# ADVRHumanoids/mpc_fatigue

Hardware: NVIDIA B200
Metric: rollout_steps_per_s_with_jacobians (higher is better)
Workload: dtype f64

## Files before the change

### mpc_fatigue_b200/csrc/kernels_jvp2.cu

```cuda
#include <atomic>
#include <cstdlib>
#include <mutex>
#include <vector>

#include "derivs.cuh"
#include "launch.cuh"

namespace mpcf {

template <int N>
struct WsLayout {
    static constexpr int kTile = 32;
    static constexpr int kPlanes2 = 3 * N * N;
    static constexpr int kPlanes1 = 4 * N;
    static constexpr int kQd = 0, kQdd = N, kFd = 2 * N, kQ = 3 * N;
    static constexpr int kStageDoubles = (kPlanes2 + kPlanes1) * kTile;
    static constexpr unsigned kStageBytes = kStageDoubles * sizeof(double);
    static constexpr int kRingDoubles = (kPlanes2 + 3 * N) * kTile;
    static constexpr unsigned kRingBytes = kRingDoubles * sizeof(double);
    static constexpr int kUnitDoubles = 4 * (kPlanes2 + kPlanes1);
    static MPCF_DI size_t chunk(long tile, int s) { return ((size_t)tile * 4 + s) * kStageDoubles; }
};
size_t jvp_ws_doubles_per_unit(int n) { return (size_t)4 * (3 * n * n + 4 * n); }

// ... 104 lines not shown
#pragma unroll
    for (int i = 0; i < N; ++i) {
        q[i] = __ldcs(w + (W::kQ + i) * 32);
        qd[i] = __ldcs(w + (W::kQd + i) * 32);
        qdd[i] = __ldcs(w + (W::kQdd + i) * 32);
    }
    {
        const long lin = (long)blockIdx.y * gridDim.x + blockIdx.x + 2 * kSmCountHint;
        if (lin < 4l * gridDim.x) {
            const long lu2 = (lin % gridDim.x) * blockDim.x + threadIdx.x;
            if (lu2 < cnt) {
                const double *o2 = ws + W::chunk(lu2 / 32, (int)(lin / gridDim.x)) + (lu2 & 31);
#pragma unroll
                for (int i = 0; i < N; ++i) {
                    asm volatile("prefetch.global.L2 [%0];" ::"l"(o2 + (W::kPlanes2 + W::kQ + i) * 32));
                    asm volatile("prefetch.global.L2 [%0];" ::"l"(o2 + (W::kPlanes2 + W::kQd + i) * 32));
                    asm volatile("prefetch.global.L2 [%0];" ::"l"(o2 + (W::kPlanes2 + W::kQdd + i) * 32));
                }
#pragma unroll
                for (int r = 0; r < N; ++r)
#pragma unroll
                    for (int c = 0; c <= r; ++c) asm volatile("prefetch.global.L2 [%0];" ::"l"(o2 + (2 * N * N + r * N + c) * 32));
            }
        }
    }
    auto emit = [&](int mat, int r, int c, double v) { __stcs(o + (mat * N * N + r * N + c) * 32, v); };
    if (KSMEM) {
        extern __shared__ double k2_slab[];
        SharedLinkStore ks{k2_slab + threadIdx.x, (int)blockDim.x};
        CFromShared Cs{k2_slab + 18 * (N - 1) * blockDim.x + threadIdx.x, (int)blockDim.x};
#pragma unroll
        for (int r = 0; r < N; ++r)
#pragma unroll
            for (int c = 0; c <= r; ++c) cp_async8(Cs.base + (r * (r + 1) / 2 + c) * Cs.stride, o + (2 * N * N + r * N + c) * 32);
        FdDerivs<StaticModel<N, L>, L>::run_cols(m, q, qd, qdd, Cs, emit, ks);
    } else {
        LocalLinkStore<N> ks;
        CFromGlobal<N> Cs{o};
        FdDerivs<StaticModel<N, L>, L>::run_cols(m, q, qd, qdd, Cs, emit, ks);
    }
}

template <int N>
__global__ void __launch_bounds__(kThreads) k_fd_derivs(const __grid_constant__ StaticParams<N> P, long U, const double *q, const double *qd,
                                                       const double *tau, double *Ao, double *Bo, double *Co, int ntot, int c0)
{
    const StaticModel<N, N> m{P};
    const long u = (long)blockIdx.x * blockDim.x + threadIdx.x;
    if (u >= U) return;
    double a[N], b[N], c[N], qdd[N], Cv[N * (N + 1) / 2];
#pragma unroll
    for (int i = 0; i < N; ++i) { a[i] = q[i * U + u]; b[i] = qd[i * U + u]; c[i] = tau[i * U + u]; }
    Dyn<double, StaticModel<N, N>>::template fd_crba<N, true>(m, a, b, c, qdd, Cv);
    auto at = [&](int r, int cc) { return (size_t)((c0 + r) * ntot + c0 + cc) * U + u; };
#pragma unroll
    for (int r = 0; r < N; ++r)
#pragma unroll
        for (int cc = 0; cc < N; ++cc) Co[at(r, cc)] = Cv[r >= cc ? r * (r + 1) / 2 + cc : cc * (cc + 1) / 2 + r];
    auto cget = [&](int r, int cc) { return Cv[r * (r + 1) / 2 + cc]; };
    CFromRegisters<decltype(cget)> Cs{cget};
    auto emit = [&](int mat, int r, int cc, double v) { (mat == 0 ? Ao : Bo)[at(r, cc)] = v; };
    extern __shared__ double link_slab[];
    SharedLinkStore ks{link_slab + threadIdx.x, (int)blockDim.x};
    FdDerivs<StaticModel<N, N>, N>::run_cols(m, a, b, qdd, Cs, emit, ks);
#pragma unroll 1
    for (int r = 0; r < N; ++r)
#pragma unroll 1
        for (int cc = 0; cc < ntot; ++cc)
            if (cc < c0 || cc >= c0 + N) {
                const size_t k = (size_t)((c0 + r) * ntot + cc) * U + u;
                Ao[k] = 0.0; Bo[k] = 0.0; Co[k] = 0.0;
            }
}

template <int N>
__global__ void __launch_bounds__(kThreads) k_rnea_derivs(const __grid_constant__ StaticParams<N> P, long U, const double *q, const double *qd,
                                                         const double *qdd, double *Dq, double *Dv, double *Mo, int ntot, int c0)
{
    const StaticModel<N, N> m{P};
    const long u = (long)blockIdx.x * blockDim.x + threadIdx.x;
    if (u >= U) return;
    double a[N], b[N], c[N];
#pragma unroll
    for (int i = 0; i < N; ++i) { a[i] = q[i * U + u]; b[i] = qd[i * U + u]; c[i] = qdd ? qdd[i * U + u] : 0.0; }
    extern __shared__ double link_slab[];
    SharedLinkStore ks{link_slab + threadIdx.x, (int)blockDim.x};
    struct Hooks {
        double *Dq, *Dv, *Mo;
        long U, u;
        int ntot, c0;
        MPCF_DI size_t at(int r, int cc) const { return (size_t)((c0 + r) * ntot + c0 + cc) * U + u; }
        MPCF_DI void link(int, const double *, const double *) const {}
        MPCF_DI void pair(int k, int j, const LinkFwd &, const LinkFwd &, double dqkj, double dqjk, double dvkj, double dvjk, double mkj) const
        {
            Dq[at(k, j)] = dqkj;
            Dv[at(k, j)] = dvkj;
            Mo[at(k, j)] = mkj;
            if (j < k) {
                Dq[at(j, k)] = dqjk;
                Dv[at(j, k)] = dvjk;
                Mo[at(j, k)] = mkj;
            }
        }
    } hooks{Dq, Dv, Mo, U, u, ntot, c0};
    FdDerivs<StaticModel<N, N>, N>::run_id_stream(m, a, b, c, hooks, ks);
#pragma unroll 1
    for (int r = 0; r < N; ++r)
#pragma unroll 1
        for (int cc = 0; cc < ntot; ++cc)
            if (cc < c0 || cc >= c0 + N) {
                const size_t k = (size_t)((c0 + r) * ntot + cc) * U + u;
                Dq[k] = 0.0; Dv[k] = 0.0; Mo[k] = 0.0;
            }
}

template <int N, int NEE>
struct NodeEvalJvpHooks {
    static constexpr int NE = NEE > 0 ? NEE : 1;
    double *Dq, *Dv;
    long U, u;
    int ntot, c0;
    double wsign;
    int je[NE];
    double pl[NE][3], pf[NE][3], Wo[NE][6];
    MPCF_DI void link(int i, const double *R, const double *o)
    {
#pragma unroll
        for (int e = 0; e < NEE; ++e)
            if (je[e] == i) {
#pragma unroll
                for (int r = 0; r < 3; ++r) pf[e][r] = o[r] + R[3 * r] * pl[e][0] + R[3 * r + 1] * pl[e][1] + R[3 * r + 2] * pl[e][2];
                double t[3];
                cross3(pf[e], Wo[e], t);
#pragma unroll
                for (int r = 0; r < 3; ++r) Wo[e][3 + r] += t[r];
            }
    }
    MPCF_DI void hvec(const LinkFwd &Kj, int e, double *h) const
    {
        double t[3], dp[3];
        cross3(Kj.S + 3, pf[e], t);
#pragma unroll
        for (int r = 0; r < 3; ++r) dp[r] = Kj.S[r] + t[r];
        cross3(dp, Wo[e], h);
    }
    MPCF_DI void pair(int k, int j, const LinkFwd &Kk, const LinkFwd &Kj, double dqkj, double dqjk, double dvkj, double dvjk, double) const
    {
#pragma unroll
        for (int e = 0; e < NEE; ++e)
            if (k <= je[e]) {
                double hj[3];
                hvec(Kj, e, hj);
                double vkj = dot3(Kk.S + 3, hj);
                if (j < k) {
                    double x[6], hk[3];
                    mxm(Kj.S, Kk.S, x);
                    vkj += dot6(x, Wo[e]);
                    hvec(Kk, e, hk);
                    dqjk += wsign * dot3(Kj.S + 3, hk);
                }
                dqkj += wsign * vkj;
            }
        Dq[(size_t)((c0 + k) * ntot + c0 + j) * U + u] = dqkj;
        Dv[(size_t)((c0 + k) * ntot + c0 + j) * U + u] = dvkj;
        if (j < k) {
            Dq[(size_t)((c0 + j) * ntot + c0 + k) * U + u] = dqjk;
            Dv[(size_t)((c0 + j) * ntot + c0 + k) * U + u] = dvjk;
        }
    }
};

template <int N, int NEE>
__global__ void __launch_bounds__(kThreads) k_node_eval_jvp(const __grid_constant__ StaticParams<N> P, long U, EeArgs ee, double wsign,
                                                           const double *q, const double *qd, const double *qdd, const double *W,
                                                           double *Dq, double *Dv, int ntot, int c0)
{
    const StaticModel<N, N> m{P};
    const long u = (long)blockIdx.x * blockDim.x + threadIdx.x;
    if (u >= U) return;
    double a[N], b[N], c[N];
#pragma unroll
    for (int i = 0; i < N; ++i) { a[i] = q[i * U + u]; b[i] = qd[i * U + u]; c[i] = qdd ? qdd[i * U + u] : 0.0; }
    NodeEvalJvpHooks<N, NEE> hooks;
    hooks.Dq = Dq; hooks.Dv = Dv; hooks.U = U; hooks.u = u; hooks.ntot = ntot; hooks.c0 = c0; hooks.wsign = wsign;
#pragma unroll
    for (int e = 0; e < NEE; ++e) {
        const int j = e < ee.nee ? ee.f[e].joint - c0 : -1;
        hooks.je[e] = (e < ee.nee && ee.f[e].joint >= 0 && j >= 0 && j < N) ? j : -1;
#pragma unroll
        for (int r = 0; r < 3; ++r) { hooks.pl[e][r] = ee.f[e].p[r]; hooks.pf[e][r] = 0.0; }
#pragma unroll
        for (int r = 0; r < 6; ++r) hooks.Wo[e][r] = (hooks.je[e] >= 0) ? W[(long)(6 * e + r) * U + u] : 0.0;
    }
    extern __shared__ double link_slab[];
    SharedLinkStore ks{link_slab + threadIdx.x, (int)blockDim.x};
    FdDerivs<StaticModel<N, N>, N>::run_id_stream(m, a, b, c, hooks, ks);
#pragma unroll 1
    for (int r = 0; r < N; ++r)
#pragma unroll 1
        for (int cc = 0; cc < ntot; ++cc)
            if (cc < c0 || cc >= c0 + N) { Dq[(size_t)((c0 + r) * ntot + cc) * U + u] = 0.0; Dv[(size_t)((c0 + r) * ntot + cc) * U + u] = 0.0; }
}

struct RneaDerivsDualBody {
    template <class MP>
    static MPCF_DI void run(const MP &m, long u, long U, const double *q, const double *qd, const double *qdd, double *Dq, double *Dv,
                            double *Mo)
    {
        constexpr int UNR = MP::kStatic ? MP::MAXN : 1;
        const int n = m.n();
        const int d = blockIdx.y;
        Dual a[MP::MAXN], b[MP::MAXN], c[MP::MAXN], t[MP::MAXN];
#pragma unroll UNR
        for (int i = 0; i < n; ++i) {
            a[i] = Dual(q[i * U + u], d == i ? 1.0 : 0.0);
            b[i] = Dual(qd[i * U + u], d == n + i ? 1.0 : 0.0);
            c[i] = Dual(qdd ? qdd[i * U + u] : 0.0, d == 2 * n + i ? 1.0 : 0.0);
        }
        Dyn<Dual, MP>::rnea(m, a, b, c, t);
        double *out = d < n ? Dq : (d < 2 * n ? Dv : Mo);
        const int col = d % n;
#pragma unroll UNR
        for (int r = 0; r < n; ++r) out[(size_t)(r * n + col) * U + u] = t[r].d;
    }
};

struct FdDerivsDualBody {
    template <class MP>
    static MPCF_DI void run(const MP &m, long u, long U, const double *q, const double *qd, const double *tau, double *Ao, double *Bo,
                            double *Co)
    {
        constexpr int UNR = MP::kStatic ? MP::MAXN : 1;
        const int n = m.n();
        const int d = blockIdx.y;
        Dual a[MP::MAXN], b[MP::MAXN], c[MP::MAXN], t[MP::MAXN];
#pragma unroll UNR
        for (int i = 0; i < n; ++i) {
            a[i] = Dual(q[i * U + u], d == i ? 1.0 : 0.0);
            b[i] = Dual(qd[i * U + u], d == n + i ? 1.0 : 0.0);
            c[i] = Dual(tau[i * U + u], d == 2 * n + i ? 1.0 : 0.0);
        }
        Dyn<Dual, MP>::aba(m, a, b, c, t);
        double *out = d < n ? Ao : (d < 2 * n ? Bo : Co);
        const int col = d % n;
#pragma unroll UNR
        for (int r = 0; r < n; ++r) out[(size_t)(r * n + col) * U + u] = t[r].d;
    }
};

template <int N, int L>
struct ColumnState {
    double Xq[N], Xv[N], Xf[N], aq[N], av[N], af[N];
    int jq, jv, jt;
    bool isdt;
    double ktau;
    double xq1;

    MPCF_DI void set_tau(const StaticParams<N> &P, double tauj)
    {
        ktau = 0.0;
#pragma unroll
        for (int i = 0; i < N; ++i)
            if (i == jt) ktau = 2.0 * P.fat[i][1] * P.fat[i][2] * tauj;
    }
    MPCF_DI void init(int col)
    {
        jq = col < N ? col : -1;
        jv = (col >= N && col < 2 * N) ? col - N : -1;
        jt = (col >= 2 * N && col < 3 * N) ? col - 2 * N : -1;
        isdt = col == 3 * N;
#pragma unroll
        for (int i = 0; i < N; ++i) {
            Xq[i] = (i == jq) ? 1.0 : 0.0;
            Xv[i] = (i == jv) ? 1.0 : 0.0;
            Xf[i] = 0.0;
            aq[i] = Xq[i]; av[i] = Xv[i]; af[i] = 0.0;
        }
        xq1 = 0.0;
    }
    MPCF_DI void finish(const StaticParams<N> &P, int s, const double *w1, double h, const double *nv)
    {
        const double cs = s < 2 ? 0.5 : (s == 2 ? 1.0 : 0.0);
        const double wt = (s == 0 || s == 3) ? 1.0 / 6.0 : 1.0 / 3.0;
#pragma unroll
        for (int i = 0; i < N; ++i) {
            const double qds = w1[(WsLayout<N>::kQd + i) * 32];
            double kf = 2.0 * P.fat[i][1] * P.fat[i][3] * qds * Xv[i] - P.fat[i][0] * Xf[i];
            if (i == jt) kf += ktau;
            double yq = h * Xv[i], yf = h * kf, yv = h * nv[i];
            if (isdt) {
                yq += qds;
                yv += w1[(WsLayout<N>::kQdd + i) * 32];
                yf += w1[(WsLayout<N>::kFd + i) * 32];
            }
            aq[i] = fma(wt, yq, aq[i]);
            av[i] = fma(wt, yv, av[i]);
            af[i] = fma(wt, yf, af[i]);
            Xq[i] = ((i == jq) ? 1.0 : 0.0) + cs * yq;
            Xv[i] = ((i == jv) ? 1.0 : 0.0) + cs * yv;
            Xf[i] = cs * yf;
            if (s == 0 && (i == jq || i == jv)) xq1 = Xq[i];
        }
    }
    MPCF_DI void stage(const StaticParams<N> &P, int s, const double *w, double h)
    {
        double nv[N];
        if (s == 0) {
#pragma unroll
            for (int r = 0; r < N; ++r) {
                double kv = 0.0;
                if (jq >= 0 && jq / L == r / L) kv = w[(r * N + jq) * 32];
                if (jv >= 0 && jv / L == r / L) kv = w[(N * N + r * N + jv) * 32];
                nv[r] = kv;
            }
        } else if (s == 1 && !isdt) {
            const int js = jq >= 0 ? jq : jv;
#pragma unroll
            for (int r = 0; r < N; ++r) {
                double kv = 0.0;
                if (js >= 0 && js / L == r / L) kv = w[(r * N + js) * 32] * xq1;
#pragma unroll
                for (int c = 0; c < N; ++c) {
                    if (r / L != c / L) continue;
                    kv = fma(w[(N * N + r * N + c) * 32], Xv[c], kv);
                }
                nv[r] = kv;
            }
        } else {
#pragma unroll
            for (int r = 0; r < N; ++r) {
                double kv = 0.0;
#pragma unroll
                for (int c = 0; c < N; ++c) {
                    if (r / L != c / L) continue;
                    kv = fma(w[(r * N + c) * 32], Xq[c], kv);
                    kv = fma(w[(N * N + r * N + c) * 32], Xv[c], kv);
                }
                nv[r] = kv;
            }
        }
        if (jt >= 0) {
#pragma unroll
            for (int r = 0; r < N; ++r)
                if (jt / L == r / L) nv[r] += w[(2 * N * N + r * N + jt) * 32];
        }
        finish(P, s, w + 3 * N * N * 32, h, nv);
    }
    static MPCF_DI void stage2(ColumnState &a, ColumnState &b, const StaticParams<N> &P, int s, const double *w, double h)
    {
        double na[N], nb[N];
#pragma unroll
        for (int r = 0; r < N; ++r) {
            double ka = 0.0, kb = 0.0;
#pragma unroll
            for (int c = 0; c < N; ++c) {
                if (r / L != c / L) continue;
                const double A = w[(r * N + c) * 32], B = w[(N * N + r * N + c) * 32];
                ka = fma(A, a.Xq[c], ka);
                kb = fma(A, b.Xq[c], kb);
                ka = fma(B, a.Xv[c], ka);
                kb = fma(B, b.Xv[c], kb);
            }
            if (a.jt >= 0 && a.jt / L == r / L) ka += w[(2 * N * N + r * N + a.jt) * 32];
            if (b.jt >= 0 && b.jt / L == r / L) kb += w[(2 * N * N + r * N + b.jt) * 32];
            na[r] = ka;
            nb[r] = kb;
        }
        a.finish(P, s, w + 3 * N * N * 32, h, na);
        b.finish(P, s, w + 3 * N * N * 32, h, nb);
    }
    template <bool WHOLE>
    MPCF_DI void store(const StaticParams<N> &P, int col, double h, long U, long u, double *jac, int ntot_, int c0_) const
    {
        const int ntot = WHOLE ? N : ntot_, c0 = WHOLE ? 0 : c0_;
        const long PC = 4 * ntot + 1;
        const long ocol = isdt ? 4 * ntot : (col / N) * ntot + c0 + col % N;
#pragma unroll
        for (int i = 0; i < N; ++i) {
            __stcs(jac + ((size_t)(c0 + i) * PC + ocol) * U + u, aq[i]);
            __stcs(jac + ((size_t)(ntot + c0 + i) * PC + ocol) * U + u, av[i]);
            __stcs(jac + ((size_t)(2 * ntot + c0 + i) * PC + ocol) * U + u, af[i]);
        }
        if (isdt) {
#pragma unroll
            for (int j = 0; j < N; ++j) {
                const double z = P.fat[j][0] * h;
                const double g = 1.0 + z * (-1.0 + z * (0.5 + z * (-1.0 / 6.0 + z * (1.0 / 24.0))));
                if (WHOLE) {
#pragma unroll
                    for (int r = 0; r < 3 * N; ++r) __stcs(jac + ((size_t)r * PC + 3 * N + j) * U + u, (r == 2 * N + j) ? g : 0.0);
                } else {
#pragma unroll
                    for (int blk = 0; blk < 3; ++blk)
#pragma unroll
                        for (int i = 0; i < N; ++i)
                            __stcs(jac + ((size_t)(blk * ntot + c0 + i) * PC + 3 * ntot + c0 + j) * U + u, (blk == 2 && i == j) ? g : 0.0);
                }
            }
        }
    }
};

template <int N, int L>
__global__ void __launch_bounds__(kThreads) k_step_vjp(const __grid_constant__ StaticParams<N> P, long U, long u0, long cnt,
                                                      const double *__restrict__ tau, double dt, const double *__restrict__ dt_u,
                                                      const VjpArgs a, int gdt_add, const double *__restrict__ ws)
{
    static_assert(N == L, "the reverse sweep runs one serial chain at a time (forests: one launch per chain)");
    using W = WsLayout<N>;
    const long lu = (long)blockIdx.x * blockDim.x + threadIdx.x;
    if (lu >= cnt) return;
    const long u = u0 + lu;
    const double h = dt_u ? dt_u[u] : dt;
    double lam[3 * N], gx[3 * N], ad[3 * N], gt[N], kt[N];
#pragma unroll
    for (int i = 0; i < N; ++i) {
        lam[i] = a.lq ? a.lq[i * a.ldl + u] : 0.0;
        lam[N + i] = a.lqd ? a.lqd[i * a.ldl + u] : 0.0;
        lam[2 * N + i] = a.lf ? a.lf[i * a.ldl + u] : 0.0;
        gx[i] = lam[i] + (a.aq ? a.aq[i * a.lda + u] : 0.0);
        gx[N + i] = lam[N + i] + (a.aqd ? a.aqd[i * a.lda + u] : 0.0);
        gx[2 * N + i] = lam[2 * N + i] + (a.af ? a.af[i * a.lda + u] : 0.0);
        kt[i] = 2.0 * P.fat[i][1] * P.fat[i][2] * tau[i * U + u];
        gt[i] = 0.0;
    }
#pragma unroll
    for (int i = 0; i < 3 * N; ++i) ad[i] = 0.0;
    double gh = 0.0;
#pragma unroll 1
    for (int s = 3; s >= 0; --s) {
        const double cs = s < 2 ? 0.5 : (s == 2 ? 1.0 : 0.0);
        const double wt = (s == 0 || s == 3) ? 1.0 / 6.0 : 1.0 / 3.0;
        const double *w = ws + W::chunk(lu / 32, s) + (lu & 31);
        const double *v = w + W::kPlanes2 * 32;
        double rq[N], rv[N], rf[N], nq[N], nv[N];
#pragma unroll
        for (int i = 0; i < N; ++i) {
            const double qds = __ldcs(v + (W::kQd + i) * 32);
            const double pq = fma(wt, lam[i], cs * ad[i]), pv = fma(wt, lam[N + i], cs * ad[N + i]),
                         pf = fma(wt, lam[2 * N + i], cs * ad[2 * N + i]);
            gh = fma(pq, qds, gh);
            gh = fma(pv, __ldcs(v + (W::kQdd + i) * 32), gh);
            gh = fma(pf, __ldcs(v + (W::kFd + i) * 32), gh);
            rq[i] = h * pq;
            rv[i] = h * pv;
            rf[i] = h * pf;
            nq[i] = 0.0;
            nv[i] = fma(2.0 * P.fat[i][1] * P.fat[i][3] * qds, rf[i], rq[i]);
            gt[i] = fma(kt[i], rf[i], gt[i]);
        }
#pragma unroll
        for (int r = 0; r < N; ++r) {
            if (P.fence0 > r) continue;
            const double x = rv[r];
#pragma unroll
            for (int c = 0; c < N; ++c) {
                nq[c] = fma(__ldcs(w + (r * N + c) * 32), x, nq[c]);
                nv[c] = fma(__ldcs(w + (N * N + r * N + c) * 32), x, nv[c]);
                gt[c] = fma(__ldcs(w + (2 * N * N + r * N + c) * 32), x, gt[c]);
            }
        }
#pragma unroll
        for (int i = 0; i < N; ++i) {
            ad[i] = nq[i];
            ad[N + i] = nv[i];
            ad[2 * N + i] = -P.fat[i][0] * rf[i];
            gx[i] += ad[i];
            gx[N + i] += ad[N + i];
            gx[2 * N + i] += ad[2 * N + i];
        }
    }
#pragma unroll
    for (int i = 0; i < N; ++i) {
        a.gq[i * a.ldg + u] = gx[i];
        a.gqd[i * a.ldg + u] = gx[N + i];
        a.gf[i * a.ldg + u] = gx[2 * N + i];
        a.gtau[i * a.ldgt + u] = gt[i];
    }
    if (a.gdt) a.gdt[u] = gdt_add ? a.gdt[u] + gh : gh;
}

MPCF_DI unsigned smem_u32(const void *p) { return (unsigned)__cvta_generic_to_shared(p); }
MPCF_DI void mbar_init(unsigned long long *bar, unsigned count)
{
    asm volatile("mbarrier.init.shared::cta.b64 [%0], %1;" ::"r"(smem_u32(bar)), "r"(count) : "memory");
}
MPCF_DI void mbar_arrive(unsigned long long *bar)
{
    asm volatile("{\n\t.reg .b64 st;\n\tmbarrier.arrive.shared::cta.b64 st, [%0];\n\t}" ::"r"(smem_u32(bar)) : "memory");
}
MPCF_DI void mbar_arrive_expect_tx(unsigned long long *bar, unsigned bytes)
{
    asm volatile("{\n\t.reg .b64 st;\n\tmbarrier.arrive.expect_tx.release.cta.shared::cta.b64 st, [%0], %1;\n\t}" ::"r"(smem_u32(bar)), "r"(bytes)
                 : "memory");
}
MPCF_DI void mbar_wait(unsigned long long *bar, unsigned parity)
{
    unsigned done;
    do {
        asm volatile("{\n\t.reg .pred p;\n\tmbarrier.try_wait.parity.shared::cta.b64 p, [%1], %2;\n\tselp.b32 %0, 1, 0, p;\n\t}"
                     : "=r"(done)
                     : "r"(smem_u32(bar)), "r"(parity)
                     : "memory");
    } while (!done);
}
MPCF_DI void bulk_g2s(void *dst, const void *src, unsigned bytes, unsigned long long *bar)
{
    asm volatile("cp.async.bulk.shared::cluster.global.mbarrier::complete_tx::bytes [%0], [%1], %2, [%3];" ::"r"(smem_u32(dst)), "l"(src),
                 "r"(bytes), "r"(smem_u32(bar))
                 : "memory");
}

template <class W, int NBUF>
MPCF_DI void tma_issue(unsigned item, double *buf, unsigned long long *full, unsigned long long *empty, const double *ws, unsigned bid,
                       unsigned nblk)
{
    const unsigned slot = item % NBUF, round = item / NBUF;
    const long t = bid + (long)(item / 4) * nblk;
    mbar_wait(&empty[slot], (round & 1) ^ 1);
    mbar_arrive_expect_tx(&full[slot], W::kRingBytes);
    bulk_g2s(buf + (size_t)slot * W::kRingDoubles, ws + W::chunk(t, item & 3), W::kRingBytes, &full[slot]);
}

template <int N, int L, int NBUF, int CPW, bool WHOLE>
__global__ void __launch_bounds__(32 * ((3 * N + CPW) / CPW), 1)
    k_chain_rule_tma(const __grid_constant__ StaticParams<N> P, long U, long u0, long cnt, const double *__restrict__ tau, long UT, double dt,
                     const double *__restrict__ dt_u, const double *__restrict__ ws, double *__restrict__ jac, long UJ, int ntot, int c0)
{
    using W = WsLayout<N>;
    constexpr int NC = 3 * N + 1;
    constexpr int NW = (NC + CPW - 1) / CPW;
    extern __shared__ __align__(128) unsigned char smem_raw[];
    double *buf = reinterpret_cast<double *>(smem_raw);
    unsigned long long *full = reinterpret_cast<unsigned long long *>(smem_raw + (size_t)NBUF * W::kRingBytes);
    unsigned long long *empty = full + NBUF;
    const int warp = threadIdx.x >> 5, lane = threadIdx.x & 31;
    const long ntiles = (cnt + 31) / 32;
    const long my_tiles = blockIdx.x < ntiles ? (ntiles - blockIdx.x + gridDim.x - 1) / gridDim.x : 0;
    const unsigned nitems = (unsigned)(my_tiles * 4);
    const bool producer = threadIdx.x == 0;
    if (producer) {
        for (int i = 0; i < NBUF; ++i) { mbar_init(&full[i], 1); mbar_init(&empty[i], NW); }
        asm volatile("fence.mbarrier_init.release.cluster;" ::: "memory");
        for (unsigned i = 0; i < NBUF - 1 && i < nitems; ++i)
            tma_issue<W, NBUF>(i, buf, full, empty, ws, blockIdx.x, gridDim.x);
    }
    __syncthreads();
    const int col0 = warp, col1 = warp + NW;
    const bool two = CPW == 2 && col1 < NC;
    unsigned it = 0;
    for (long t = blockIdx.x; t < ntiles; t += gridDim.x) {
        const long lu = t * 32 + lane;
        const bool live = lu < cnt;
        const long u = u0 + (live ? lu : 0);
        const double h = dt_u ? dt_u[u] : dt;
        ColumnState<N, L> a, b;
        a.init(col0);
        a.set_tau(P, a.jt >= 0 ? tau[(size_t)a.jt * UT + u] : 0.0);
        if (CPW == 2) {
            b.init(two ? col1 : col0);
            b.set_tau(P, b.jt >= 0 ? tau[(size_t)b.jt * UT + u] : 0.0);
        }
#pragma unroll 1
        for (int s = 0; s < 4; ++s, ++it) {
            if (producer && it + NBUF - 1 < nitems) tma_issue<W, NBUF>(it + NBUF - 1, buf, full, empty, ws, blockIdx.x, gridDim.x);
            const unsigned slot = it % NBUF, round = it / NBUF;
            mbar_wait(&full[slot], round & 1);
            const double *w = buf + (size_t)slot * W::kRingDoubles + lane;
            if (CPW == 2) ColumnState<N, L>::stage2(a, b, P, s, w, h);
            else a.stage(P, s, w, h);
            __syncwarp();
            if (lane == 0) mbar_arrive(&empty[slot]);
        }
        if (live) {
            a.template store<WHOLE>(P, col0, h, UJ, u, jac, ntot, c0);
            if (two) b.template store<WHOLE>(P, col1, h, UJ, u, jac, ntot, c0);
        }
    }
}

template <int N, int L, int NCY>
__global__ void __launch_bounds__(32 * NCY, 2)
    k_chain_rule_ldg(const __grid_constant__ StaticParams<N> P, long U, long u0, long cnt, const double *__restrict__ tau, long UT, double dt,
                     const double *__restrict__ dt_u, const double *__restrict__ ws, double *__restrict__ jac, long UJ, int ntot, int c0)
{
    using W = WsLayout<N>;
    const long lu = (long)blockIdx.x * 32 + threadIdx.x;
    if (lu >= cnt) return;
    const long u = u0 + lu;
    const double h = dt_u ? dt_u[u] : dt;
    constexpr int NC = 3 * N + 1;
    for (int col = threadIdx.y; col < NC; col += blockDim.y) {
        ColumnState<N, L> st;
        st.init(col);
        st.set_tau(P, st.jt >= 0 ? tau[(size_t)st.jt * UT + u] : 0.0);
#pragma unroll 1
        for (int s = 0; s < 4; ++s) st.stage(P, s, ws + W::chunk(blockIdx.x, s) + threadIdx.x, h);
        st.template store<false>(P, col, h, UJ, u, jac, ntot, c0);
    }
}

struct ProfEvent { cudaEvent_t a, b; int k; };
static std::atomic<bool> g_prof_on{false};
static std::mutex g_prof_mu;
static std::vector<ProfEvent> g_prof;
void jvp_profile_enable(bool on) { g_prof_on.store(on); }
static cudaEvent_t prof_begin(int k, cudaStream_t s)
{
    if (!g_prof_on.load(std::memory_order_relaxed)) return nullptr;
    ProfEvent e;
    cudaEventCreate(&e.a);
    cudaEventCreate(&e.b);
    e.k = k;
    cudaEventRecord(e.a, s);
    std::lock_guard<std::mutex> lk(g_prof_mu);
    g_prof.push_back(e);
    return e.b;
}
static void prof_end(cudaEvent_t b, cudaStream_t s)
{
    if (b) cudaEventRecord(b, s);
}
int jvp_profile_read(double *ms3, long *launches)
{
    std::lock_guard<std::mutex> lk(g_prof_mu);
    ms3[0] = ms3[1] = ms3[2] = 0.0;
    *launches = (long)g_prof.size();
    for (auto &e : g_prof) {
        float t = 0.f;
        cudaEventSynchronize(e.b);
        cudaEventElapsedTime(&t, e.a, e.b);
        ms3[e.k] += t;
        cudaEventDestroy(e.a);
        cudaEventDestroy(e.b);
    }
    g_prof.clear();
    return 0;
}

static int current_device()
{
    int dev = 0;
    cudaGetDevice(&dev);
    return dev >= 0 && dev < 64 ? dev : 0;
}
static int sm_count()
{
    static int n[64] = {};
    const int dev = current_device();
    if (!n[dev]) {
        cudaDeviceGetAttribute(&n[dev], cudaDevAttrMultiProcessorCount, dev);
        if (n[dev] <= 0) n[dev] = 148;
    }
    return n[dev];
}

template <int N, int L>
struct K2Config {
    static constexpr int kThreadsK2 = (2 * (18 * (N - 1) + N * (N + 1) / 2) * kThreads * (int)sizeof(double) <= 227 * 1024) ? kThreads : 96;
    static constexpr int kSlab = (18 * (N - 1) + N * (N + 1) / 2) * kThreadsK2 * (int)sizeof(double);
    static constexpr bool kSmem = N == L && 2 * kSlab <= 227 * 1024;
};

template <int N, int L>
static void launch_stages_derivs(const StaticParams<N> &P, long U, long u0, long cnt, const double *q, const double *qd, const double *tau,
                                 const double *theat, long UT, const double *f, double dt, const double *dt_u, double *qn, double *qdn,
                                 double *fn, double *ws, cudaStream_t s)
{
    using K2 = K2Config<N, L>;
    const unsigned gb = (unsigned)((cnt + kThreads - 1) / kThreads);
    cudaEvent_t pe = prof_begin(0, s);
    k_step_stages<N, L><<<gb, kThreads, 0, s>>>(P, U, u0, cnt, q, qd, tau, theat, UT, f, dt, dt_u, qn, qdn, fn, ws);
    prof_end(pe, s);
    pe = prof_begin(1, s);
    static const int k2smem = getenv("MPCF_K2_SMEM") ? atoi(getenv("MPCF_K2_SMEM")) : 1;
    bool k2done = false;
    if constexpr (K2::kSmem) {
        if (k2smem) {
            k_stage_derivs<N, L, true><<<dim3((unsigned)((cnt + K2::kThreadsK2 - 1) / K2::kThreadsK2), 4), K2::kThreadsK2, K2::kSlab, s>>>(P, cnt, ws);
            k2done = true;
        }
    }
    if (!k2done) k_stage_derivs<N, L, false><<<dim3(gb, 4), kThreads, 0, s>>>(P, cnt, ws);
    prof_end(pe, s);
}

template <int N, int L>
static cudaError_t run_jvp2(const StaticParams<N> &P, long U, long Ucnt, const double *q, const double *qd, const double *tau, const double *theat,
                            long UT, const double *f,
                            double dt, const double *dt_u, double *qn, double *qdn, double *fn, double *jac, long UJ, double *ws, long Uc,
                            cudaStream_t s, int ntot = N, int c0 = 0)
{
    using W = WsLayout<N>;
    constexpr bool kTma = N <= 7;
    constexpr int kRingMax = (227 * 1024 - 256) / (int)W::kRingBytes;
    constexpr int NBUF = kTma ? (kRingMax > 5 ? 5 : kRingMax) : 0;
    constexpr int kCpwDefault = (3 * N + 1 <= 19) ? 1 : 2;
    constexpr size_t smem = (size_t)NBUF * W::kRingBytes + 2 * NBUF * sizeof(unsigned long long);
    using K2 = K2Config<N, L>;
    constexpr bool kK2Smem = K2::kSmem;
    if constexpr (kTma) {
        static std::atomic<bool> attr_set[64];
        const int dev = current_device();
        if (!attr_set[dev].load(std::memory_order_acquire)) {
            cudaError_t e = cudaSuccess;
            if constexpr (kCpwDefault == 1) {
                e = cudaFuncSetAttribute(k_chain_rule_tma<N, L, NBUF, 1, true>, cudaFuncAttributeMaxDynamicSharedMemorySize, (int)smem);
                if (e != cudaSuccess) return e;
                e = cudaFuncSetAttribute(k_chain_rule_tma<N, L, NBUF, 1, false>, cudaFuncAttributeMaxDynamicSharedMemorySize, (int)smem);
                if (e != cudaSuccess) return e;
            }
            e = cudaFuncSetAttribute(k_chain_rule_tma<N, L, NBUF, 2, true>, cudaFuncAttributeMaxDynamicSharedMemorySize, (int)smem);
            if (e != cudaSuccess) return e;
            e = cudaFuncSetAttribute(k_chain_rule_tma<N, L, NBUF, 2, false>, cudaFuncAttributeMaxDynamicSharedMemorySize, (int)smem);
            if (e != cudaSuccess) return e;
            if constexpr (kK2Smem) {
                e = cudaFuncSetAttribute(k_stage_derivs<N, L, true>, cudaFuncAttributeMaxDynamicSharedMemorySize, K2::kSlab);
                if (e != cudaSuccess) return e;
            }
            attr_set[dev].store(true, std::memory_order_release);
        }
    }
    for (long u0 = 0; u0 < Ucnt; u0 += Uc) {
        const long cnt = (Ucnt - u0) < Uc ? (Ucnt - u0) : Uc;
        const long ntiles = (cnt + 31) / 32;
        launch_stages_derivs<N, L>(P, U, u0, cnt, q, qd, tau, theat, UT, f, dt, dt_u, qn, qdn, fn, ws, s);
        cudaEvent_t pe = prof_begin(2, s);
        if constexpr (kTma) {
            const unsigned g3 = (unsigned)(ntiles < sm_count() ? ntiles : sm_count());
            static const int cpw_env = getenv("MPCF_K3_CPW") ? atoi(getenv("MPCF_K3_CPW")) : 1;
            const int cpw = kCpwDefault == 2 ? 2 : cpw_env;
            if (cpw == 2) {
                (ntot == N ? k_chain_rule_tma<N, L, NBUF, 2, true> : k_chain_rule_tma<N, L, NBUF, 2, false>)<<<g3, 32 * ((3 * N + 2) / 2), smem, s>>>(
                    P, U, u0, cnt, theat, UT, dt, dt_u, ws, jac, UJ, ntot, c0);
            } else if constexpr (kCpwDefault == 1) {
                (ntot == N ? k_chain_rule_tma<N, L, NBUF, 1, true> : k_chain_rule_tma<N, L, NBUF, 1, false>)<<<g3, 32 * (3 * N + 1), smem, s>>>(
                    P, U, u0, cnt, theat, UT, dt, dt_u, ws, jac, UJ, ntot, c0);
            }
        } else {
            k_chain_rule_ldg<N, L, 10><<<(unsigned)ntiles, dim3(32, 10), 0, s>>>(P, U, u0, cnt, theat, UT, dt, dt_u, ws, jac, UJ, ntot, c0);
        }
        prof_end(pe, s);
        g_launches.fetch_add(3);
    }
    return cudaGetLastError();
}

template <int L, class V>
__global__ void __launch_bounds__(256) k_forest_fill_cross(int ntot, long cntv, long UJ, double *jac)
{
    const long uv = (long)blockIdx.x * blockDim.x + threadIdx.x;
    if (uv >= cntv) return;
    const int r = blockIdx.y, rc = (r % ntot) / L, nch = ntot / L;
    const long PC = 4 * ntot + 1;
    V zero;
    memset(&zero, 0, sizeof(V));
    double *row = jac + (size_t)r * PC * UJ;
    for (int b = 0; b < 4; ++b)
        for (int oc = 0; oc < nch; ++oc) {
            if (oc == rc) continue;
            double *p = row + (size_t)(b * ntot + oc * L) * UJ;
#pragma unroll
            for (int i = 0; i < L; ++i) __stcs(reinterpret_cast<V *>(p + (size_t)i * UJ) + uv, zero);
        }
}

template <int L>
static cudaError_t run_forest(const LaunchModel &m, long U, long Ucnt, const double *q, const double *qd, const double *tau, const double *theat,
                              long UT, const double *f, double dt,
                              const double *dt_u, double *qn, double *qdn, double *fn, double *jac, long UJ, double *ws, long Uc, cudaStream_t s)
{
    const StaticParams<L> *cp = static_cast<const StaticParams<L> *>(m.chain_params);
    for (int c = 0; c < m.n / L; ++c) {
        const size_t off = (size_t)c * L * U;
        cudaError_t e = run_jvp2<L, L>(cp[c], U, Ucnt, q + off, qd + off, tau + off, theat + (size_t)c * L * UT, UT, f + off, dt, dt_u, qn ? qn + off : nullptr,
                                       qdn ? qdn + off : nullptr, fn ? fn + off : nullptr, jac, UJ, ws, Uc, s, m.n, L * c);
        if (e != cudaSuccess) return e;
    }
    if (Ucnt % 2 == 0 && UJ % 2 == 0 && (reinterpret_cast<size_t>(jac) & 15) == 0)
        k_forest_fill_cross<L, double2><<<dim3((unsigned)((Ucnt / 2 + 255) / 256), 3 * m.n), 256, 0, s>>>(m.n, Ucnt / 2, UJ, jac);
    else
        k_forest_fill_cross<L, double><<<dim3((unsigned)((Ucnt + 255) / 256), 3 * m.n), 256, 0, s>>>(m.n, Ucnt, UJ, jac);
    g_launches.fetch_add(1);
    return cudaGetLastError();
}

bool jvp2_supported(const LaunchModel &m) { return family_chain_len(m.fam) > 0; }

cudaError_t launch_step_jvp_ws(const LaunchModel &m, long U, const double *q, const double *qd, const double *tau, const double *f,
                               double dt, const double *dt_u, double *qn, double *qdn, double *fn, double *jac, double *ws,
                               size_t ws_bytes, cudaStream_t s, long cnt, long UJ, const double *theat, long UT)
{
    if (!theat) { theat = tau; UT = U; }
    if (cnt < 0) cnt = U;
    if (UJ <= 0) UJ = U;
    if (cnt <= 0) return cudaSuccess;
    const size_t per_unit = jvp_ws_doubles_per_unit(family_chain_len(m.fam)) * sizeof(double);
    long Uc = (long)(ws_bytes / per_unit);
    Uc -= Uc % 32;
    if (Uc < 32) return cudaErrorInvalidValue;
    switch (m.fam) {
    case FAM_CHAIN3:
        return run_jvp2<3, 3>(*static_cast<const StaticParams<3> *>(m.static_params), U, cnt, q, qd, tau, theat, UT, f, dt, dt_u, qn, qdn, fn, jac, UJ, ws, Uc, s);
    case FAM_CHAIN6:
        return run_jvp2<6, 6>(*static_cast<const StaticParams<6> *>(m.static_params), U, cnt, q, qd, tau, theat, UT, f, dt, dt_u, qn, qdn, fn, jac, UJ, ws, Uc, s);
    case FAM_CHAIN7:
        return run_jvp2<7, 7>(*static_cast<const StaticParams<7> *>(m.static_params), U, cnt, q, qd, tau, theat, UT, f, dt, dt_u, qn, qdn, fn, jac, UJ, ws, Uc, s);
    case FAM_FOREST12x6:
        return run_forest<6>(m, U, cnt, q, qd, tau, theat, UT, f, dt, dt_u, qn, qdn, fn, jac, UJ, ws, Uc, s);
    case FAM_FOREST14x7:
        return run_forest<7>(m, U, cnt, q, qd, tau, theat, UT, f, dt, dt_u, qn, qdn, fn, jac, UJ, ws, Uc, s);
    default:
        return cudaErrorInvalidValue;
    }
}

template <int N, int L>
static cudaError_t run_vjp2(const StaticParams<N> &P, long U, long Ucnt, const double *q, const double *qd, const double *tau, const double *f,
                            double dt, const double *dt_u, const VjpArgs &a, int gdt_add, double *qn, double *qdn, double *fn, double *ws, long Uc,
                            cudaStream_t s)
{
    using K2 = K2Config<N, L>;
    if constexpr (K2::kSmem) {
        static std::atomic<bool> attr_set[64];
        const int dev = current_device();
        if (!attr_set[dev].load(std::memory_order_acquire)) {
            const cudaError_t e = cudaFuncSetAttribute(k_stage_derivs<N, L, true>, cudaFuncAttributeMaxDynamicSharedMemorySize, K2::kSlab);
            if (e != cudaSuccess) return e;
            attr_set[dev].store(true, std::memory_order_release);
        }
    }
    for (long u0 = 0; u0 < Ucnt; u0 += Uc) {
        const long cnt = (Ucnt - u0) < Uc ? (Ucnt - u0) : Uc;
        launch_stages_derivs<N, L>(P, U, u0, cnt, q, qd, tau, tau, U, f, dt, dt_u, qn, qdn, fn, ws, s);
        k_step_vjp<N, L><<<(unsigned)((cnt + kThreads - 1) / kThreads), kThreads, 0, s>>>(P, U, u0, cnt, tau, dt, dt_u, a, gdt_add, ws);
        g_launches.fetch_add(3);
    }
    return cudaGetLastError();
}

template <int L>
static cudaError_t vjp_chains(const LaunchModel &m, long U, long cnt, const double *q, const double *qd, const double *tau, const double *f,
                              double dt, const double *dt_u, const VjpArgs &a, double *qn, double *qdn, double *fn, double *ws, long Uc,
                              cudaStream_t s)
{
    const StaticParams<L> *cp = static_cast<const StaticParams<L> *>(m.n == L ? m.static_params : m.chain_params);
    for (int c = 0; c < m.n / L; ++c) {
        const size_t off = (size_t)c * L * U;
        const cudaError_t e = run_vjp2<L, L>(cp[c], U, cnt, q + off, qd + off, tau + off, f + off, dt, dt_u, a.rows(c * L), c > 0,
                                             qn ? qn + off : nullptr, qdn ? qdn + off : nullptr, fn ? fn + off : nullptr, ws, Uc, s);
        if (e != cudaSuccess) return e;
    }
    return cudaSuccess;
}

cudaError_t launch_step_vjp_ws(const LaunchModel &m, long U, long cnt, const double *q, const double *qd, const double *tau, const double *f,
                               double dt, const double *dt_u, const VjpArgs &a, double *qn, double *qdn, double *fn, double *ws,
                               size_t ws_bytes, cudaStream_t s)
{
    if (cnt <= 0) return cudaSuccess;
    const size_t per_unit = jvp_ws_doubles_per_unit(family_chain_len(m.fam)) * sizeof(double);
    long Uc = (long)(ws_bytes / per_unit);
    Uc -= Uc % 32;
    if (Uc < 32) return cudaErrorInvalidValue;
    switch (family_chain_len(m.fam)) {
    case 3: return vjp_chains<3>(m, U, cnt, q, qd, tau, f, dt, dt_u, a, qn, qdn, fn, ws, Uc, s);
    case 6: return vjp_chains<6>(m, U, cnt, q, qd, tau, f, dt, dt_u, a, qn, qdn, fn, ws, Uc, s);
    case 7: return vjp_chains<7>(m, U, cnt, q, qd, tau, f, dt, dt_u, a, qn, qdn, fn, ws, Uc, s);
    default: return cudaErrorInvalidValue;
    }
}

static constexpr int link_slab_bytes(int n) { return 18 * (n - 1) * kThreads * (int)sizeof(double); }

template <int L>
static cudaError_t node_eval_jvp_chains(const LaunchModel &m, const EeArgs &ee, double wsign, long U, const double *q, const double *qd,
                                        const double *qdd, const double *W, double *dtau_dq, double *dtau_dqd, cudaStream_t s)
{
    const unsigned gb = (unsigned)((U + kThreads - 1) / kThreads);
    const StaticParams<L> *cp = static_cast<const StaticParams<L> *>(m.n == L ? m.static_params : m.chain_params);
    for (int c = 0; c < m.n / L; ++c) {
        const size_t off = (size_t)c * L * U;
        auto go = [&](auto kern) {
            cudaError_t e = cudaFuncSetAttribute(kern, cudaFuncAttributeMaxDynamicSharedMemorySize, link_slab_bytes(L));
            if (e != cudaSuccess) return e;
            kern<<<gb, kThreads, link_slab_bytes(L), s>>>(cp[c], U, ee, wsign, q + off, qd + off, qdd ? qdd + off : nullptr, W, dtau_dq, dtau_dqd,
                                                         m.n, c * L);
            return cudaSuccess;
        };
        const cudaError_t e = ee.nee == 0 ? go(k_node_eval_jvp<L, 0>) : ee.nee == 1 ? go(k_node_eval_jvp<L, 1>)
                              : ee.nee == 2 ? go(k_node_eval_jvp<L, 2>) : go(k_node_eval_jvp<L, MPCF_MAX_EE>);
        if (e != cudaSuccess) return e;
        g_launches.fetch_add(1);
    }
    return cudaGetLastError();
}

cudaError_t launch_node_eval_jvp(const LaunchModel &m, const EeArgs &ee, double wsign, long U, const double *q, const double *qd,
                                 const double *qdd, const double *W, double *dtau_dq, double *dtau_dqd, cudaStream_t s)
{
    if (U <= 0) return cudaSuccess;
    switch (family_chain_len(m.fam)) {
    case 3: return node_eval_jvp_chains<3>(m, ee, wsign, U, q, qd, qdd, W, dtau_dq, dtau_dqd, s);
    case 6: return node_eval_jvp_chains<6>(m, ee, wsign, U, q, qd, qdd, W, dtau_dq, dtau_dqd, s);
    case 7: return node_eval_jvp_chains<7>(m, ee, wsign, U, q, qd, qdd, W, dtau_dq, dtau_dqd, s);
    default: return launch_node_eval_jvp_dual(m, ee, wsign, U, q, qd, qdd, W, dtau_dq, dtau_dqd, s);
    }
}

template <int L>
static cudaError_t rnea_derivs_chains(const LaunchModel &m, long U, const double *q, const double *qd, const double *qdd, double *Dq, double *Dv,
                                      double *M, cudaStream_t s)
{
    const unsigned gb = (unsigned)((U + kThreads - 1) / kThreads);
    const StaticParams<L> *cp = static_cast<const StaticParams<L> *>(m.n == L ? m.static_params : m.chain_params);
    const cudaError_t e = cudaFuncSetAttribute(k_rnea_derivs<L>, cudaFuncAttributeMaxDynamicSharedMemorySize, link_slab_bytes(L));
    if (e != cudaSuccess) return e;
    for (int c = 0; c < m.n / L; ++c) {
        const size_t off = (size_t)c * L * U;
        k_rnea_derivs<L><<<gb, kThreads, link_slab_bytes(L), s>>>(cp[c], U, q + off, qd + off, qdd ? qdd + off : nullptr, Dq, Dv, M, m.n, c * L);
        g_launches.fetch_add(1);
    }
    return cudaGetLastError();
}

cudaError_t launch_rnea_derivs(const LaunchModel &m, long U, const double *q, const double *qd, const double *qdd, double *Dq, double *Dv,
                               double *M, cudaStream_t s)
{
    if (U <= 0) return cudaSuccess;
    switch (family_chain_len(m.fam)) {
    case 3: return rnea_derivs_chains<3>(m, U, q, qd, qdd, Dq, Dv, M, s);
    case 6: return rnea_derivs_chains<6>(m, U, q, qd, qdd, Dq, Dv, M, s);
    case 7: return rnea_derivs_chains<7>(m, U, q, qd, qdd, Dq, Dv, M, s);
    default: return dispatch_generic<RneaDerivsDualBody>(m, U, 3 * m.n, s, q, qd, qdd, Dq, Dv, M);
    }
}

template <int L>
static cudaError_t fd_derivs_chains(const LaunchModel &m, long U, const double *q, const double *qd, const double *tau, double *A, double *B,
                                    double *C, cudaStream_t s)
{
    const unsigned gb = (unsigned)((U + kThreads - 1) / kThreads);
    const StaticParams<L> *cp = static_cast<const StaticParams<L> *>(m.n == L ? m.static_params : m.chain_params);
    const cudaError_t e = cudaFuncSetAttribute(k_fd_derivs<L>, cudaFuncAttributeMaxDynamicSharedMemorySize, link_slab_bytes(L));
    if (e != cudaSuccess) return e;
    for (int c = 0; c < m.n / L; ++c) {
        const size_t off = (size_t)c * L * U;
        k_fd_derivs<L><<<gb, kThreads, link_slab_bytes(L), s>>>(cp[c], U, q + off, qd + off, tau + off, A, B, C, m.n, c * L);
        g_launches.fetch_add(1);
    }
    return cudaGetLastError();
}

cudaError_t launch_fd_derivs(const LaunchModel &m, long U, const double *q, const double *qd, const double *tau, double *A, double *B,
                             double *C, cudaStream_t s)
{
    if (U <= 0) return cudaSuccess;
    switch (family_chain_len(m.fam)) {
    case 3: return fd_derivs_chains<3>(m, U, q, qd, tau, A, B, C, s);
    case 6: return fd_derivs_chains<6>(m, U, q, qd, tau, A, B, C, s);
    case 7: return fd_derivs_chains<7>(m, U, q, qd, tau, A, B, C, s);
    default: return dispatch_generic<FdDerivsDualBody>(m, U, 3 * m.n, s, q, qd, tau, A, B, C);
    }
}

}
```

Measured before the change: 226.0 million.

## Fuse stage-derivative and chain-rule kernels for six-joint serial chains

New measurement: 240.1 million, median of 6. 6.3% higher.

```diff
diff --git a/mpc_fatigue_b200/csrc/kernels_jvp2.cu b/mpc_fatigue_b200/csrc/kernels_jvp2.cu
--- a/mpc_fatigue_b200/csrc/kernels_jvp2.cu
+++ b/mpc_fatigue_b200/csrc/kernels_jvp2.cu
@@ -430,7 +430,9 @@
             if (s == 0 && (i == jq || i == jv)) xq1 = Xq[i];
         }
     }
-    MPCF_DI void stage(const StaticParams<N> &P, int s, const double *w, double h)
+    MPCF_DI void stage(const StaticParams<N> &P, int s, const double *w, double h) { stage(P, s, w, CFromGlobal<N>{w}, w + 3 * N * N * 32, h); }
+    template <class CM>
+    MPCF_DI void stage(const StaticParams<N> &P, int s, const double *w, const CM &Cm, const double *wv, double h)
     {
         double nv[N];
         if (s == 0) {
@@ -470,9 +472,9 @@
         if (jt >= 0) {
 #pragma unroll
             for (int r = 0; r < N; ++r)
-                if (jt / L == r / L) nv[r] += w[(2 * N * N + r * N + jt) * 32];
-        }
-        finish(P, s, w + 3 * N * N * 32, h, nv);
+                if (jt / L == r / L) nv[r] += Cm(r, jt);
+        }
+        finish(P, s, wv, h, nv);
     }
     static MPCF_DI void stage2(ColumnState &a, ColumnState &b, const StaticParams<N> &P, int s, const double *w, double h)
     {
@@ -497,7 +499,7 @@
         a.finish(P, s, w + 3 * N * N * 32, h, na);
         b.finish(P, s, w + 3 * N * N * 32, h, nb);
     }
-    template <bool WHOLE>
+    template <bool WHOLE, bool FCOLS = true>
     MPCF_DI void store(const StaticParams<N> &P, int col, double h, long U, long u, double *jac, int ntot_, int c0_) const
     {
         const int ntot = WHOLE ? N : ntot_, c0 = WHOLE ? 0 : c0_;
@@ -509,21 +511,26 @@
             __stcs(jac + ((size_t)(ntot + c0 + i) * PC + ocol) * U + u, av[i]);
             __stcs(jac + ((size_t)(2 * ntot + c0 + i) * PC + ocol) * U + u, af[i]);
         }
-        if (isdt) {
-#pragma unroll
-            for (int j = 0; j < N; ++j) {
-                const double z = P.fat[j][0] * h;
-                const double g = 1.0 + z * (-1.0 + z * (0.5 + z * (-1.0 / 6.0 + z * (1.0 / 24.0))));
-                if (WHOLE) {
-#pragma unroll
-                    for (int r = 0; r < 3 * N; ++r) __stcs(jac + ((size_t)r * PC + 3 * N + j) * U + u, (r == 2 * N + j) ? g : 0.0);
-                } else {
-#pragma unroll
-                    for (int blk = 0; blk < 3; ++blk)
-#pragma unroll
-                        for (int i = 0; i < N; ++i)
-                            __stcs(jac + ((size_t)(blk * ntot + c0 + i) * PC + 3 * ntot + c0 + j) * U + u, (blk == 2 && i == j) ? g : 0.0);
-                }
+        if (FCOLS && isdt) fatigue_cols<WHOLE>(P, h, U, u, jac, ntot, c0);
+    }
+    template <bool WHOLE>
+    static MPCF_DI void fatigue_cols(const StaticParams<N> &P, double h, long U, long u, double *jac, int ntot_, int c0_)
+    {
+        const int ntot = WHOLE ? N : ntot_, c0 = WHOLE ? 0 : c0_;
+        const long PC = 4 * ntot + 1;
+#pragma unroll
+        for (int j = 0; j < N; ++j) {
+            const double z = P.fat[j][0] * h;
+            const double g = 1.0 + z * (-1.0 + z * (0.5 + z * (-1.0 / 6.0 + z * (1.0 / 24.0))));
+            if (WHOLE) {
+#pragma unroll
+                for (int r = 0; r < 3 * N; ++r) __stcs(jac + ((size_t)r * PC + 3 * N + j) * U + u, (r == 2 * N + j) ? g : 0.0);
+            } else {
+#pragma unroll
+                for (int blk = 0; blk < 3; ++blk)
+#pragma unroll
+                    for (int i = 0; i < N; ++i)
+                        __stcs(jac + ((size_t)(blk * ntot + c0 + i) * PC + 3 * ntot + c0 + j) * U + u, (blk == 2 && i == j) ? g : 0.0);
             }
         }
     }
@@ -728,6 +735,111 @@
     }
 }
 
+template <int N>
+struct FusedLayout {
+    static constexpr int kLinkPlanes = 18 * (N - 1);
+    static constexpr int kTri = N * (N + 1) / 2;
+    static constexpr int kSlab = (kLinkPlanes + kTri) * kThreads * (int)sizeof(double);
+    static constexpr int kStage = (2 * N * N + 3 * N) * 32;
+    static constexpr bool kFits = 4 * kStage <= kLinkPlanes * kThreads;
+};
+
+template <int N, int L, bool WHOLE>
+__global__ void __launch_bounds__(kThreads) k_stage_derivs_chain(const __grid_constant__ StaticParams<N> P, long U, long u0, long cnt,
+                                                                 const double *__restrict__ tau, long UT, double dt, const double *__restrict__ dt_u,
+                                                                 double *ws, double *__restrict__ jac, long UJ, int ntot, int c0)
+{
+    static_assert(N == L && FusedLayout<N>::kFits, "one serial chain whose four stages fit the link slab");
+    static_assert(kThreads == 128, "one warp per RK4 stage");
+    const StaticModel<N, L> m{P};
+    using W = WsLayout<N>;
+    using F = FusedLayout<N>;
+    extern __shared__ __align__(128) double fused_slab[];
+    __shared__ unsigned long long full[4];
+    const int s = threadIdx.x >> 5, lane = threadIdx.x & 31;
+    const long lu = (long)blockIdx.x * 32 + lane;
+    const bool live = lu < cnt;
+    const int lc = live ? lane : (int)((cnt - 1) & 31);
+    double *o = ws + W::chunk(blockIdx.x, s) + lane;
+    const double *in = ws + W::chunk(blockIdx.x, s) + lc;
+    if (threadIdx.x == 0) {
+#pragma unroll
+        for (int i = 0; i < 4; ++i) mbar_init(&full[i], 1);
+        asm volatile("fence.mbarrier_init.release.cluster;" ::: "memory");
+    }
+    double q[N], qd[N], qdd[N];
+#pragma unroll
+    for (int i = 0; i < N; ++i) {
+        q[i] = __ldcs(in + (W::kPlanes2 + W::kQ + i) * 32);
+        qd[i] = __ldcs(in + (W::kPlanes2 + W::kQd + i) * 32);
+        qdd[i] = __ldcs(in + (W::kPlanes2 + W::kQdd + i) * 32);
+    }
+    {
+        const long t2 = (long)blockIdx.x + 2 * kSmCountHint;
+        const long lu2 = t2 * 32 + lane;
+        if (t2 < gridDim.x && lu2 < cnt) {
+            const double *o2 = ws + W::chunk(t2, s) + lane;
+#pragma unroll
+            for (int i = 0; i < 4 * N; ++i) asm volatile("prefetch.global.L2 [%0];" ::"l"(o2 + (W::kPlanes2 + i) * 32));
+#pragma unroll
+            for (int r = 0; r < N; ++r)
+#pragma unroll
+                for (int c = 0; c <= r; ++c) asm volatile("prefetch.global.L2 [%0];" ::"l"(o2 + (2 * N * N + r * N + c) * 32));
+        }
+    }
+    CFromShared Cs{fused_slab + F::kLinkPlanes * kThreads + threadIdx.x, kThreads};
+    {
+        SharedLinkStore ks{fused_slab + threadIdx.x, kThreads};
+#pragma unroll
+        for (int r = 0; r < N; ++r)
+#pragma unroll
+            for (int c = 0; c <= r; ++c) cp_async8(Cs.base + (r * (r + 1) / 2 + c) * kThreads, in + (2 * N * N + r * N + c) * 32);
+        auto emit = [&](int mat, int r, int c, double v) { o[(mat * N * N + r * N + c) * 32] = v; };
+        FdDerivs<StaticModel<N, L>, L>::run_cols(m, q, qd, qdd, Cs, emit, ks);
+    }
+    asm volatile("fence.proxy.async;" ::: "memory");
+    __syncthreads();
+    if (threadIdx.x == 0) {
+        asm volatile("fence.proxy.async;" ::: "memory");
+#pragma unroll
+        for (int st = 0; st < 4; ++st) {
+            const double *src = ws + W::chunk(blockIdx.x, st);
+            double *dst = fused_slab + st * F::kStage;
+            mbar_arrive_expect_tx(&full[st], F::kStage * (unsigned)sizeof(double));
+            bulk_g2s(dst, src, 2 * N * N * 32 * (unsigned)sizeof(double), &full[st]);
+            bulk_g2s(dst + 2 * N * N * 32, src + W::kPlanes2 * 32, 3 * N * 32 * (unsigned)sizeof(double), &full[st]);
+        }
+    }
+    constexpr int NC = 3 * N + 1;
+    const long u = u0 + (long)blockIdx.x * 32 + lc;
+    const double h = dt_u ? dt_u[u] : dt;
+#pragma unroll 1
+    for (int col = s; col < NC; col += 4) {
+        ColumnState<N, L> a;
+        a.init(col);
+        a.set_tau(P, a.jt >= 0 ? tau[(size_t)a.jt * UT + u] : 0.0);
+#pragma unroll 1
+        for (int st = 0; st < 4; ++st) {
+            mbar_wait(&full[st], 0);
+            const CFromShared Ct{fused_slab + F::kLinkPlanes * kThreads + st * 32 + lane, kThreads};
+            auto Cm = [&](int r, int c) { return r >= c ? Ct(r, c) : Ct(c, r); };
+            const double *w = fused_slab + st * F::kStage + lane;
+            a.stage(P, st, w, Cm, w + 2 * N * N * 32, h);
+        }
+        if (live) a.template store<WHOLE, false>(P, col, h, UJ, u, jac, ntot, c0);
+    }
+}
+
+template <int N, bool WHOLE>
+__global__ void __launch_bounds__(kThreads) k_fatigue_cols(const __grid_constant__ StaticParams<N> P, long u0, long cnt, double dt,
+                                                           const double *__restrict__ dt_u, double *jac, long UJ, int ntot, int c0)
+{
+    const long lu = (long)blockIdx.x * blockDim.x + threadIdx.x;
+    if (lu >= cnt) return;
+    const long u = u0 + lu;
+    ColumnState<N, N>::template fatigue_cols<WHOLE>(P, dt_u ? dt_u[u] : dt, UJ, u, jac, ntot, c0);
+}
+
 struct ProfEvent { cudaEvent_t a, b; int k; };
 static std::atomic<bool> g_prof_on{false};
 static std::mutex g_prof_mu;
@@ -791,16 +903,25 @@
 };
 
 template <int N, int L>
+static void launch_step_stages(const StaticParams<N> &P, long U, long u0, long cnt, const double *q, const double *qd, const double *tau,
+                               const double *theat, long UT, const double *f, double dt, const double *dt_u, double *qn, double *qdn,
+                               double *fn, double *ws, cudaStream_t s)
+{
+    cudaEvent_t pe = prof_begin(0, s);
+    k_step_stages<N, L><<<(unsigned)((cnt + kThreads - 1) / kThreads), kThreads, 0, s>>>(P, U, u0, cnt, q, qd, tau, theat, UT, f, dt, dt_u, qn,
+                                                                                      qdn, fn, ws);
+    prof_end(pe, s);
+}
+
+template <int N, int L>
 static void launch_stages_derivs(const StaticParams<N> &P, long U, long u0, long cnt, const double *q, const double *qd, const double *tau,
                                  const double *theat, long UT, const double *f, double dt, const double *dt_u, double *qn, double *qdn,
                                  double *fn, double *ws, cudaStream_t s)
 {
     using K2 = K2Config<N, L>;
     const unsigned gb = (unsigned)((cnt + kThreads - 1) / kThreads);
-    cudaEvent_t pe = prof_begin(0, s);
-    k_step_stages<N, L><<<gb, kThreads, 0, s>>>(P, U, u0, cnt, q, qd, tau, theat, UT, f, dt, dt_u, qn, qdn, fn, ws);
-    prof_end(pe, s);
-    pe = prof_begin(1, s);
+    launch_step_stages<N, L>(P, U, u0, cnt, q, qd, tau, theat, UT, f, dt, dt_u, qn, qdn, fn, ws, s);
+    cudaEvent_t pe = prof_begin(1, s);
     static const int k2smem = getenv("MPCF_K2_SMEM") ? atoi(getenv("MPCF_K2_SMEM")) : 1;
     bool k2done = false;
     if constexpr (K2::kSmem) {
@@ -827,6 +948,7 @@
     constexpr size_t smem = (size_t)NBUF * W::kRingBytes + 2 * NBUF * sizeof(unsigned long long);
     using K2 = K2Config<N, L>;
     constexpr bool kK2Smem = K2::kSmem;
+    constexpr bool kFused = N == 6 && kK2Smem && FusedLayout<N>::kFits;
     if constexpr (kTma) {
         static std::atomic<bool> attr_set[64];
         const int dev = current_device();
@@ -846,12 +968,36 @@
                 e = cudaFuncSetAttribute(k_stage_derivs<N, L, true>, cudaFuncAttributeMaxDynamicSharedMemorySize, K2::kSlab);
                 if (e != cudaSuccess) return e;
             }
+            if constexpr (kFused) {
+                for (auto kern : {k_stage_derivs_chain<N, L, true>, k_stage_derivs_chain<N, L, false>}) {
+                    e = cudaFuncSetAttribute(kern, cudaFuncAttributeMaxDynamicSharedMemorySize, FusedLayout<N>::kSlab);
+                    if (e != cudaSuccess) return e;
+                }
+            }
             attr_set[dev].store(true, std::memory_order_release);
         }
     }
+    const char *fused_env = getenv("MPCF_JVP_FUSED");
+    const bool fused = kFused && !(fused_env && atoi(fused_env) == 0);
     for (long u0 = 0; u0 < Ucnt; u0 += Uc) {
         const long cnt = (Ucnt - u0) < Uc ? (Ucnt - u0) : Uc;
         const long ntiles = (cnt + 31) / 32;
+        if constexpr (kFused) {
+            if (fused) {
+                launch_step_stages<N, L>(P, U, u0, cnt, q, qd, tau, theat, UT, f, dt, dt_u, qn, qdn, fn, ws, s);
+                cudaEvent_t pe = prof_begin(1, s);
+                const bool whole = ntot == N;
+                (whole ? k_stage_derivs_chain<N, L, true> : k_stage_derivs_chain<N, L, false>)<<<(unsigned)ntiles, kThreads, FusedLayout<N>::kSlab, s>>>(
+                    P, U, u0, cnt, theat, UT, dt, dt_u, ws, jac, UJ, ntot, c0);
+                prof_end(pe, s);
+                pe = prof_begin(2, s);
+                (whole ? k_fatigue_cols<N, true> : k_fatigue_cols<N, false>)<<<(unsigned)((cnt + kThreads - 1) / kThreads), kThreads, 0, s>>>(
+                    P, u0, cnt, dt, dt_u, jac, UJ, ntot, c0);
+                prof_end(pe, s);
+                g_launches.fetch_add(3);
+                continue;
+            }
+        }
         launch_stages_derivs<N, L>(P, U, u0, cnt, q, qd, tau, theat, UT, f, dt, dt_u, qn, qdn, fn, ws, s);
         cudaEvent_t pe = prof_begin(2, s);
         if constexpr (kTma) {
diff --git a/profiles/fused_jvp_timing.py b/profiles/fused_jvp_timing.py
--- /dev/null
+++ b/profiles/fused_jvp_timing.py
@@ -0,0 +1,119 @@
+import argparse
+import ctypes as C
+import json
+import os
+import statistics
+import subprocess
+import sys
+
+ROOT = os.path.dirname(os.path.dirname(os.path.abspath(__file__)))
+if ROOT not in sys.path:
+    sys.path.insert(0, ROOT)
+
+import torch
+
+from mpc_fatigue_b200 import _capi
+from mpc_fatigue_b200.evaluator import BatchEvaluator
+from mpc_fatigue_b200.model import Model, data_urdf
+from mpc_fatigue_b200.synth import synth_batch
+
+PATHS = {"fused": "1", "unfused": "0"}
+
+
+def device_info():
+    try:
+        out = subprocess.run(["nvidia-smi", "-i", str(torch.cuda.current_device()),
+                              "--query-gpu=power.limit,clocks.sm,clocks.max.sm", "--format=csv,noheader"],
+                             capture_output=True, text=True, timeout=30).stdout.strip()
+    except (OSError, subprocess.SubprocessError) as e:
+        out = "unavailable (%s)" % e
+    return {"device": torch.cuda.get_device_name(0), "power_limit, sm_clock, max_sm_clock": out}
+
+
+def make_case(name):
+    if name == "C2":
+        m, B, N = Model.from_urdf(data_urdf("pilz6"), armature=1e-2), 65536, 100
+    elif name == "C3":
+        from mpc_fatigue_b200.coupling import box_load_coupling
+        m, B, N = Model.from_urdf(data_urdf("pilz6x2"), armature=1e-2), 16384, 100
+        m.set_coupling(box_load_coupling(m))
+    elif name == "chain3":
+        m, B, N = Model.from_urdf(data_urdf("pilz3"), armature=1e-2), 65536, 100
+    else:
+        raise ValueError(name)
+    lim = {k: m.export(k) for k in ("q_lo", "q_hi", "v_max", "tau_max")}
+    return m, synth_batch(lim, 0, B, N, seed=1234, device="cuda"), B * N
+
+
+def run_path(path, fn):
+    os.environ["MPCF_JVP_FUSED"] = PATHS[path]
+    fn()
+
+
+def timed(path, fn, calls):
+    os.environ["MPCF_JVP_FUSED"] = PATHS[path]
+    fn()
+    torch.cuda.synchronize()
+    e0, e1 = torch.cuda.Event(enable_timing=True), torch.cuda.Event(enable_timing=True)
+    e0.record()
+    for _ in range(calls):
+        fn()
+    e1.record()
+    torch.cuda.synchronize()
+    return e0.elapsed_time(e1) / calls
+
+
+def kernel_split(path, fn):
+    os.environ["MPCF_JVP_FUSED"] = PATHS[path]
+    torch.cuda.synchronize()
+    _capi.lib.mpcf_profile_enable(1)
+    fn()
+    torch.cuda.synchronize()
+    ms3, nlaunch = (C.c_double * 3)(), C.c_long()
+    _capi.lib.mpcf_profile_read(ms3, C.byref(nlaunch))
+    _capi.lib.mpcf_profile_enable(0)
+    return {"K1_ms": round(ms3[0], 3), "K2_or_fused_ms": round(ms3[1], 3), "K3_ms": round(ms3[2], 3), "bracketed_launches": nlaunch.value}
+
+
+def case(name, rounds, calls, dt=0.02):
+    m, inputs, U = make_case(name)
+    ev = BatchEvaluator(m)
+    n = m.n
+    res = {p: [torch.empty((n, U), dtype=torch.float64, device="cuda") for _ in range(3)] for p in PATHS}
+    jac = {p: torch.empty((3 * n, 4 * n + 1, U), dtype=torch.float64, device="cuda") for p in PATHS}
+    fns = {p: (lambda p=p: ev.step_rk4_jvp(*inputs, dt, out=res[p], jac=jac[p])) for p in PATHS}
+    for p in PATHS:
+        run_path(p, fns[p])
+    torch.cuda.synchronize()
+    same = {nm: bool(torch.equal(a, b)) for nm, a, b in zip(("q+", "qd+", "f+"), res["fused"], res["unfused"])}
+    same["jac"] = bool(torch.equal(jac["fused"], jac["unfused"]))
+    times = {p: [] for p in PATHS}
+    for r in range(rounds):
+        for p in (("fused", "unfused") if r % 2 == 0 else ("unfused", "fused")):
+            times[p].append(timed(p, fns[p], calls))
+    out = {"case": name, "family": m.kernel_family, "units": U, "bit_identical": same}
+    for p in PATHS:
+        t = times[p]
+        out[p] = {"ms_median": round(statistics.median(t), 3), "ms_min": round(min(t), 3), "ms_max": round(max(t), 3),
+                  "spread_pct": round(100 * (max(t) - min(t)) / statistics.median(t), 2), "per_kernel": kernel_split(p, fns[p])}
+    out["fused_vs_unfused"] = round(out["fused"]["ms_median"] / out["unfused"]["ms_median"], 4)
+    del jac, res
+    torch.cuda.empty_cache()
+    return out
+
+
+def main():
+    ap = argparse.ArgumentParser()
+    ap.add_argument("--rounds", type=int, default=5)
+    ap.add_argument("--calls", type=int, default=3)
+    ap.add_argument("--cases", default="C2,C3,chain3")
+    a = ap.parse_args()
+    assert torch.cuda.is_available(), "needs a CUDA device"
+    print(json.dumps(device_info()), flush=True)
+    for name in a.cases.split(","):
+        print(json.dumps(case(name, a.rounds, a.calls)), flush=True)
+    print(json.dumps(device_info()), flush=True)
+
+
+if __name__ == "__main__":
+    main()
```
